# Edresson/VoiceSplit

Hardware: AMD Instinct MI355X
Metric: utterances/sec (3 s clips, B=64/GPU) fwd+bwd, channels-last bf16 activations / tape, bf16 MFMA, fp32 accumulate / statistics / master weights (higher is better)
Workload: dtype bf16 (conv activations and tape stored as bf16; bf16 MFMA operands in the convs, the LSTM / head contractions and the BPTT, f16 operands in the forward recurrence; fp32 accumulate, BatchNorm statistics, gate arithmetic / cell state, loss head, master weights)

## Files before the change

### voicesplit_amd/csrc/conv_nhwc.hip

```cpp
#include <utility>

#include "vs_internal.h"

namespace {

typedef unsigned u4v __attribute__((ext_vector_type(4)));
typedef unsigned u2v __attribute__((ext_vector_type(2)));
typedef float f2v __attribute__((ext_vector_type(2)));
constexpr float kLog2e = 1.44269504088896340736f;
typedef __attribute__((address_space(3))) unsigned char lds_byte;
typedef __attribute__((address_space(3))) const u4v lds_u4v;


constexpr int STRIP = 32;
constexpr int NB = STRIP / 16;
constexpr int R = 8;
#ifndef VS_NHWC_SGB
#define VS_NHWC_SGB 0
#endif

struct NhwcConvArgs {
  const unsigned short* in;
  const unsigned short* wpk;
  const float* scale;
  const float* shift;
  unsigned short* out;
  double* bn_stats;
  const unsigned short* z2;
  const float* bn2_scale; const float* bn2_shift; const float* bn2_mean; const float* bn2_invstd;
  int B, T, F, dil;
  int nstrip, nseg, seg_rows, n_items;
  unsigned* turn;
};

__device__ __forceinline__ int swz(int p) { return ((p >> 1) & 3) << 1; }

template <int KT, int KF>
struct Geo {
  static constexpr int P = KT / 2, PF = KF / 2, H = KT - 1;
  static constexpr int NTAP = KT * KF;
  static constexpr int RWPX = STRIP + 2 * PF;
  static constexpr int CPR = (RWPX * 8 + 63) / 64;
  static constexpr int ROWB = CPR * 1024;
  static constexpr int WIN = R + H;
  static constexpr int WBUF = WIN * ROWB;
  static constexpr int LDS_BYTES = 2 * WBUF;
  static constexpr int UNITS = (WIN + 3) / 4;
};

struct Item { int b, cls, strip, o0, o1, in_end, ngroups; };

template <int KT, int KF, int ACT, bool STATS, bool DY = false>
struct ConvWalk {
  using G = Geo<KT, KF>;
  static constexpr int P = G::P, PF = G::PF, H = G::H, NTAP = G::NTAP;
  static constexpr unsigned kOob = 0x7FFFFFF0u;

  const NhwcConvArgs& a;
  int lane, wave, n, g;
  vs_bf16x8 wf[NTAP][2];
  f2v csc[2], csh[2], a1[2], a2[2];
  int boff[KF][2];
  unsigned vcol[NB];
  int vdma;
  __amdgpu_buffer_rsrc_t rout, rz;
  f32x4 cacc[3][NB];
  unsigned crow[3];
  unsigned cvcol[NB];
  float ccok[NB];
  __amdgpu_buffer_rsrc_t crout, crz;
  u2v zq3[3][NB];
  unsigned lds0;
  const lds_byte* smem;

  __device__ __forceinline__ ConvWalk(const NhwcConvArgs& a_, const lds_byte* smem_) : a(a_), smem(smem_) {
    const int tid = threadIdx.x;
    lane = tid & 63;
    wave = __builtin_amdgcn_readfirstlane(tid >> 6);
    n = lane & 15;
    g = lane >> 4;
    lds0 = (unsigned)(uintptr_t)smem_;
    const u4v* wp = reinterpret_cast<const u4v*>(a.wpk) + (size_t)wave * NTAP * 2 * 64 + lane;
#pragma unroll
    for (int tap = 0; tap < NTAP; ++tap)
#pragma unroll
      for (int kc = 0; kc < 2; ++kc) wf[tap][kc] = __builtin_bit_cast(vs_bf16x8, wp[(tap * 2 + kc) * 64]);
#pragma unroll
    for (int r = 0; r < 4; ++r) {
      const int ch = wave * 16 + g * 4 + r;
      csc[r >> 1][r & 1] = DY ? a.bn2_scale[ch] * kLog2e : a.scale[ch];
      csh[r >> 1][r & 1] = DY ? a.bn2_shift[ch] * kLog2e : a.shift[ch];
      a1[r >> 1][r & 1] = 0.f;
      a2[r >> 1][r & 1] = 0.f;
    }
#pragma unroll
    for (int df = 0; df < KF; ++df) {
      const int p = n + df;
      boff[df][0] = p * 128 + ((g ^ swz(p)) << 4);
      boff[df][1] = boff[df][0] ^ 64;
    }
#pragma unroll
    for (int j = 0; j < 3; ++j) {
      crow[j] = kOob;
#pragma unroll
      for (int nb2 = 0; nb2 < NB; ++nb2) { cacc[j][nb2] = f32x4{0.f, 0.f, 0.f, 0.f}; zq3[j][nb2] = u2v{0u, 0u}; }
    }
#pragma unroll
    for (int nb2 = 0; nb2 < NB; ++nb2) { cvcol[nb2] = kOob; ccok[nb2] = 0.f; }
    crout = __builtin_amdgcn_make_buffer_rsrc(reinterpret_cast<unsigned char*>(a.out), 0, 0, 0x00020000);
    crz = crout;
    {
      const int px = lane >> 3;
      vdma = (px - PF) * 128 + (((lane & 7) ^ swz(px)) << 4);
    }
  }

  __device__ __forceinline__ bool decode(int it, Item& r) const {
    r.strip = it % a.nstrip;
    const int t1 = it / a.nstrip;
    const int seg = t1 % a.nseg;
    const int t2 = t1 / a.nseg;
    r.cls = t2 % a.dil;
    r.b = t2 / a.dil;
    const int nk = r.cls < a.T ? (a.T - r.cls + a.dil - 1) / a.dil : 0;
    r.o0 = seg * a.seg_rows;
    r.o1 = min(nk, r.o0 + a.seg_rows);
    if (r.o0 >= r.o1) return false;
    r.in_end = nk;
    r.ngroups = (r.o1 - r.o0 + R - 1) / R;
    return true;
  }

  struct Batch {
    long long row0;
    int in_end, w_first, buf, live;
    unsigned v0, v1;
  };
  Batch bt;
  __device__ __forceinline__ void begin(Batch& bt, const Item& x, int w_first, int buf) const {
    bt.row0 = (long long)x.b * a.T + x.cls;
    bt.in_end = x.in_end; bt.w_first = w_first; bt.buf = buf; bt.live = 1;
    bt.v0 = (unsigned)(vdma + ((x.strip * STRIP) << 7));
    bt.v1 = bt.v0 + 1024u;
  }
  template <int J>
  __device__ __forceinline__ void row_unit(const Batch& bt) const {
    const int rho = wave + 4 * J;
    if (!bt.live || rho >= G::WIN) return;
    const int w = bt.w_first + rho;
    const bool ok = (w >= 0) & (w < bt.in_end);
    const unsigned long long p = reinterpret_cast<unsigned long long>(a.in) + (unsigned long long)(((bt.row0 + (long long)w * a.dil) * a.F) << 7);
    const u4v d = {(unsigned)p, (unsigned)(p >> 32) & 0xffffu, ok ? (unsigned)a.F * 128u : 0u, 0x00020000u};
    const unsigned dst = lds0 + (unsigned)(bt.buf * G::WBUF + rho * G::ROWB);
    unsigned keep;
    static_assert(G::CPR == 4 || G::CPR == 5, "a window row is 4 or 5 chunks");
    if (G::CPR == 5)
      asm volatile("s_mov_b32 %0, m0\n\ts_mov_b32 m0, %3\n\ts_nop 0\n\tbuffer_load_dwordx4 %1, %2, 0 offen lds\n\t"
                   "s_add_u32 m0, %3, 0x400\n\ts_nop 0\n\tbuffer_load_dwordx4 %4, %2, 0 offen lds\n\t"
                   "buffer_load_dwordx4 %4, %2, 0 offen offset:1024 lds\n\tbuffer_load_dwordx4 %4, %2, 0 offen offset:2048 lds\n\t"
                   "buffer_load_dwordx4 %4, %2, 0 offen offset:3072 lds\n\ts_mov_b32 m0, %0"
                   : "=&s"(keep) : "v"(bt.v0), "s"(d), "s"(dst), "v"(bt.v1) : "memory", "scc");
    else
      asm volatile("s_mov_b32 %0, m0\n\ts_mov_b32 m0, %3\n\ts_nop 0\n\tbuffer_load_dwordx4 %1, %2, 0 offen lds\n\t"
                   "s_add_u32 m0, %3, 0x400\n\ts_nop 0\n\tbuffer_load_dwordx4 %4, %2, 0 offen lds\n\t"
                   "buffer_load_dwordx4 %4, %2, 0 offen offset:1024 lds\n\tbuffer_load_dwordx4 %4, %2, 0 offen offset:2048 lds\n\ts_mov_b32 m0, %0"
                   : "=&s"(keep) : "v"(bt.v0), "s"(d), "s"(dst), "v"(bt.v1) : "memory", "scc");
  }
  template <int... Js>
  __device__ __forceinline__ void all_units(const Batch& bt, std::integer_sequence<int, Js...>) const { (row_unit<Js>(bt), ...); }
  __device__ __forceinline__ void fetch_all(const Batch& bt) const { all_units(bt, std::make_integer_sequence<int, G::UNITS>()); }

  __device__ __forceinline__ void begin_item(const Item& x) {
    const size_t ub = (size_t)x.b * a.T * a.F * 128;
    const unsigned bytes = (unsigned)a.T * a.F * 128;
    rout = __builtin_amdgcn_make_buffer_rsrc(reinterpret_cast<unsigned char*>(a.out) + ub, 0, bytes, 0x00020000);
    if (DY) rz = __builtin_amdgcn_make_buffer_rsrc(const_cast<unsigned char*>(reinterpret_cast<const unsigned char*>(a.z2)) + ub, 0, bytes, 0x00020000);
#pragma unroll
    for (int nb2 = 0; nb2 < NB; ++nb2) {
      const int col = x.strip * STRIP + nb2 * 16 + n;
      vcol[nb2] = col < a.F ? (unsigned)(col * 128 + wave * 32 + g * 8) : kOob;
    }
  }
  __device__ __forceinline__ unsigned row_offset(const Item& x, int k) const {
    unsigned off;
    asm("s_mul_i32 %0, %1, %2" : "=s"(off) : "s"(x.cls + k * a.dil), "s"(a.F * 128));
    return k < x.o1 ? off : kOob;
  }

  template <int RV>
  struct GroupState {
    f32x4 acc[RV][NB];
    vs_bf16x8 bq[3];
    f2v y[NB][2];
    float cok[NB], mk[NB];
    f2v tz, ty, tu, tn, tr, tw, tp, tq;
    u2v pk[NB];
    unsigned vb[KF][2];
    int ro;
  };
  static constexpr int NSTAGE = DY ? (ACT == VS_ACT_MISH ? 19 : 7) : ACT == VS_ACT_MISH ? 12 : ACT == VS_ACT_RELU ? 2 : STATS ? 4 : 1;
  static constexpr int NMICRO = (DY ? 1 : 0) + NB * 2 * NSTAGE + 2 * NB;

  template <int RV>
  __device__ __forceinline__ vs_bf16x8 frag(const GroupState<RV>& st, int gi) const {
    const int nb = gi % NB, kc = (gi / NB) % 2, df = (gi / (2 * NB)) % KF, i = gi / (2 * NB * KF);
    return __builtin_bit_cast(vs_bf16x8, *(lds_u4v*)(uintptr_t)(st.vb[df][kc] + (unsigned)(i * G::ROWB + nb * 2048)));
  }

  static __device__ __forceinline__ float i_fma(float a, float b, float c) { return __builtin_fmaf(a, b, c); }
  static __device__ __forceinline__ float i_mul(float a, float b) { return a * b; }
  static __device__ __forceinline__ float i_add(float a, float b) { return a + b; }
  static __device__ __forceinline__ float i_add2(float a) { return a + 2.0f; }
  static __device__ __forceinline__ float i_exp2(float a) { return __builtin_amdgcn_exp2f(a); }
  static __device__ __forceinline__ float i_rcp(float a) { return __builtin_amdgcn_rcpf(a); }
  static __device__ __forceinline__ float i_max0(float a) { return fmaxf(a, 0.f); }
  static __device__ __forceinline__ float i_min_20log2e(float a) { return fminf(a, 20.0f * kLog2e); }
  static __device__ __forceinline__ float i_min_20(float a) { return fminf(a, 20.0f); }
  static __device__ __forceinline__ float i_mul_log2e(float a) { return a * kLog2e; }
  static __device__ __forceinline__ float i_mul_4ln2(float a) { return a * (4.0f * 0.69314718055994530942f); }
  static __device__ __forceinline__ float i_bf_lo(unsigned u) { return __uint_as_float(u << 16); }
  static __device__ __forceinline__ float i_bf_hi(unsigned u) { return __uint_as_float(u & 0xffff0000u); }

  static constexpr int epi_rows(int RV) { return RV >= 4 ? RV : 3; }
  template <int RV, int IDX, int nb2, int e>
  __device__ __forceinline__ float acc_of(GroupState<RV>& st) const {
    if constexpr (IDX < 3) return cacc[IDX][nb2][e];
    else return st.acc[IDX - 3][nb2][e];
  }
  template <int RV, int IDX>
  __device__ __forceinline__ unsigned rowoff_of(const Item& x, const GroupState<RV>& st) const {
    if constexpr (IDX < 3) return crow[IDX];
    else return row_offset(x, st.ro + IDX - 3);
  }
  template <int IDX, int nb2>
  __device__ __forceinline__ unsigned vcol_of() const {
    if constexpr (IDX < 3) return cvcol[nb2];
    else return vcol[nb2];
  }
  template <int RV, int IDX, bool FLUSH>
  __device__ __forceinline__ void prefetch_z(const Item& x, GroupState<RV>& st) {
    constexpr int t = IDX + 2, P_ = epi_rows(RV);
    if constexpr (t == 2) {
#pragma unroll
      for (int nb2 = 0; nb2 < NB; ++nb2) zq3[2][nb2] = __builtin_bit_cast(u2v, __builtin_amdgcn_raw_buffer_load_b64(crz, cvcol[nb2], crow[2], 0));
    } else if constexpr (!FLUSH) {
      constexpr int row = t < P_ ? t - 3 : (RV >= 4 ? RV - 3 : 0) + (t - P_);
      const unsigned so = row_offset(x, st.ro + row);
#pragma unroll
      for (int nb2 = 0; nb2 < NB; ++nb2) zq3[t % 3][nb2] = __builtin_bit_cast(u2v, __builtin_amdgcn_raw_buffer_load_b64(rz, vcol[nb2], so, 0));
    }
  }

  template <int RV, int IDX, int q, bool FLUSH>
  __device__ __forceinline__ void epi(const Item& x, GroupState<RV>& st) {
    constexpr bool mish = ACT == VS_ACT_MISH;
    constexpr int Q0 = DY ? 1 : 0;
    constexpr bool carried = IDX < 3;
    constexpr int r = IDX - 3;
    if constexpr (DY && q == 0) {
      prefetch_z<RV, IDX, FLUSH>(x, st);
#pragma unroll
      for (int nb2 = 0; nb2 < NB; ++nb2) {
        if constexpr (carried) st.mk[nb2] = crow[IDX] != kOob ? ccok[nb2] : 0.f;
        else st.mk[nb2] = (st.ro + r < x.o1) ? st.cok[nb2] : 0.f;
      }
    } else if constexpr (q < Q0 + NB * 2 * NSTAGE) {
      constexpr int v = (q - Q0) / NSTAGE, sg = (q - Q0) % NSTAGE, nb2 = v / 2, pr = v % 2;
      const float acc0 = acc_of<RV, IDX, nb2, 2 * pr>(st), acc1 = acc_of<RV, IDX, nb2, 2 * pr + 1>(st);
      if constexpr (DY) {
        if constexpr (sg == 0) {
          const unsigned u = zq3[IDX % 3][nb2][pr];
          st.tz.x = i_bf_lo(u); st.tz.y = i_bf_hi(u);
        } else if constexpr (sg == 1) {
          st.ty.x = i_fma(st.tz.x, csc[pr].x, csh[pr].x); st.ty.y = i_fma(st.tz.y, csc[pr].y, csh[pr].y);
        } else if constexpr (mish) {
          if constexpr (sg == 2) { st.ty.x = i_min_20log2e(st.ty.x); st.ty.y = i_min_20log2e(st.ty.y); }
          else if constexpr (sg == 3) st.tu.x = i_exp2(st.ty.x);
          else if constexpr (sg == 4) st.tu.y = i_exp2(st.ty.y);
          else if constexpr (sg == 5) { st.tw.x = i_add2(st.tu.x); st.tw.y = i_add2(st.tu.y); }
          else if constexpr (sg == 6) { st.tn.x = i_mul(st.tu.x, st.tw.x); st.tn.y = i_mul(st.tu.y, st.tw.y); }
          else if constexpr (sg == 7) { st.tw.x = i_add2(st.tn.x); st.tw.y = i_add2(st.tn.y); }
          else if constexpr (sg == 8) st.tr.x = i_rcp(st.tw.x);
          else if constexpr (sg == 9) st.tr.y = i_rcp(st.tw.y);
          else if constexpr (sg == 10) { st.tp.x = i_fma(st.tu.x, st.tu.x, st.tu.x); st.tp.y = i_fma(st.tu.y, st.tu.y, st.tu.y); }
          else if constexpr (sg == 11) { st.tp.x = i_mul(st.tp.x, st.ty.x); st.tp.y = i_mul(st.tp.y, st.ty.y); }
          else if constexpr (sg == 12) { st.tq.x = i_mul_4ln2(st.tr.x); st.tq.y = i_mul_4ln2(st.tr.y); }
          else if constexpr (sg == 13) { st.tn.x = i_fma(st.tp.x, st.tq.x, st.tn.x); st.tn.y = i_fma(st.tp.y, st.tq.y, st.tn.y); }
          else if constexpr (sg == 14) { st.tw.x = i_mul(st.tr.x, st.tn.x); st.tw.y = i_mul(st.tr.y, st.tn.y); }
          else if constexpr (sg == 15) { st.ty.x = i_mul(acc0, st.tw.x); st.ty.y = i_mul(acc1, st.tw.y); }
          else if constexpr (sg == 16) { st.tp.x = i_mul(st.ty.x, st.mk[nb2]); st.tp.y = i_mul(st.ty.y, st.mk[nb2]); }
          else if constexpr (sg == 17) { a1[pr].x = i_add(a1[pr].x, st.tp.x); a1[pr].y = i_add(a1[pr].y, st.tp.y); }
          else {
            a2[pr].x = i_fma(st.tp.x, st.tz.x, a2[pr].x); a2[pr].y = i_fma(st.tp.y, st.tz.y, a2[pr].y);
            st.y[nb2][pr] = st.ty;
          }
        } else {
          if constexpr (sg == 2) st.ty.x = st.ty.x > 0.f ? acc0 : 0.f;
          else if constexpr (sg == 3) st.ty.y = st.ty.y > 0.f ? acc1 : 0.f;
          else if constexpr (sg == 4) { st.tp.x = i_mul(st.ty.x, st.mk[nb2]); st.tp.y = i_mul(st.ty.y, st.mk[nb2]); }
          else if constexpr (sg == 5) { a1[pr].x = i_add(a1[pr].x, st.tp.x); a1[pr].y = i_add(a1[pr].y, st.tp.y); }
          else {
            a2[pr].x = i_fma(st.tp.x, st.tz.x, a2[pr].x); a2[pr].y = i_fma(st.tp.y, st.tz.y, a2[pr].y);
            st.y[nb2][pr] = st.ty;
          }
        }
      } else {
        if constexpr (sg == 0) {
          st.y[nb2][pr].x = i_fma(acc0, csc[pr].x, csh[pr].x); st.y[nb2][pr].y = i_fma(acc1, csc[pr].y, csh[pr].y);
        } else if constexpr (mish) {
          if constexpr (sg == 1) { st.ty.x = i_min_20(st.y[nb2][pr].x); st.ty.y = i_min_20(st.y[nb2][pr].y); }
          else if constexpr (sg == 2) { st.ty.x = i_mul_log2e(st.ty.x); st.ty.y = i_mul_log2e(st.ty.y); }
          else if constexpr (sg == 3) st.tu.x = i_exp2(st.ty.x);
          else if constexpr (sg == 4) st.tu.y = i_exp2(st.ty.y);
          else if constexpr (sg == 5) { st.tw.x = i_add2(st.tu.x); st.tw.y = i_add2(st.tu.y); }
          else if constexpr (sg == 6) { st.tn.x = i_mul(st.tu.x, st.tw.x); st.tn.y = i_mul(st.tu.y, st.tw.y); }
          else if constexpr (sg == 7) { st.tw.x = i_add2(st.tn.x); st.tw.y = i_add2(st.tn.y); }
          else if constexpr (sg == 8) st.tr.x = i_rcp(st.tw.x);
          else if constexpr (sg == 9) st.tr.y = i_rcp(st.tw.y);
          else if constexpr (sg == 10) { st.tn.x = i_mul(st.tn.x, st.tr.x); st.tn.y = i_mul(st.tn.y, st.tr.y); }
          else { st.y[nb2][pr].x = i_mul(st.y[nb2][pr].x, st.tn.x); st.y[nb2][pr].y = i_mul(st.y[nb2][pr].y, st.tn.y); }
        } else if constexpr (ACT == VS_ACT_RELU) {
          st.y[nb2][pr].x = i_max0(st.y[nb2][pr].x); st.y[nb2][pr].y = i_max0(st.y[nb2][pr].y);
        } else if constexpr (STATS) {
          if constexpr (sg == 1) {
            const float m = (int(rowoff_of<RV, IDX>(x, st) != kOob) & int(vcol_of<IDX, nb2>() != kOob)) ? 1.f : 0.f;
            st.tp.x = i_mul(st.y[nb2][pr].x, m); st.tp.y = i_mul(st.y[nb2][pr].y, m);
          } else if constexpr (sg == 2) { a1[pr].x = i_add(a1[pr].x, st.tp.x); a1[pr].y = i_add(a1[pr].y, st.tp.y); }
          else { a2[pr].x = i_fma(st.tp.x, st.y[nb2][pr].x, a2[pr].x); a2[pr].y = i_fma(st.tp.y, st.y[nb2][pr].y, a2[pr].y); }
        }
      }
    } else {
      constexpr int sq = q - Q0 - NB * 2 * NSTAGE, nb2 = sq / 2;
      if constexpr (sq % 2 == 0) {
        st.pk[nb2] = u2v{vs_pack_bf16(st.y[nb2][0].x, st.y[nb2][0].y), vs_pack_bf16(st.y[nb2][1].x, st.y[nb2][1].y)};
      } else {
        if constexpr (carried) __builtin_amdgcn_raw_buffer_store_b64(st.pk[nb2], crout, cvcol[nb2], crow[IDX], 0);
        else __builtin_amdgcn_raw_buffer_store_b64(st.pk[nb2], rout, vcol[nb2], row_offset(x, st.ro + r), 0);
      }
    }
  }

  static constexpr int nm_of(int RV, int i) { return (i < RV - 1 ? i : RV - 1) - (i - (KT - 1) > 0 ? i - (KT - 1) : 0) + 1; }
  static constexpr int slot_base(int RV, int i) { int s = 0; for (int k = 0; k < i; ++k) s += 2 * NB * KF * nm_of(RV, k); return s; }
  template <int RV>
  struct Plan {
    static constexpr int NSLOT = slot_base(RV, RV + H);
    static constexpr int P_ = epi_rows(RV);
    static constexpr int L = P_ * NMICRO;
    struct Tab { short lo[NSLOT + 1]; };
    static constexpr Tab make() {
      Tab t{};
      int c = 0, s = 0;
      for (int i = 0; i < RV + H; ++i) {
        int rows = i - H;
        if (rows < 0) rows = 0;
        if (rows > P_ - 3) rows = P_ - 3;
        const int avail = (3 + rows) * NMICRO;
        for (int k = 0; k < 2 * NB * KF * nm_of(RV, i); ++k) {
          t.lo[s] = (short)c;
          const int left = NSLOT - s;
          int want = (L - c + left - 1) / left;
          if (want < 1) want = 1;
          int n = avail - c;
          if (n > want) n = want;
          if (n < 0) n = 0;
          c += n;
          ++s;
        }
      }
      t.lo[NSLOT] = (short)c;
      return t;
    }
    static constexpr Tab tab = make();
  };
  template <int RV, bool FLUSH, int M0, int... Ds>
  __device__ __forceinline__ void epis(const Item& x, GroupState<RV>& st, std::integer_sequence<int, Ds...>) {
    (epi<RV, (M0 + Ds) / NMICRO, (M0 + Ds) % NMICRO, FLUSH>(x, st), ...);
  }

  template <int RV, int GI, int MM>
  __device__ __forceinline__ void gmfma(const Item& x, GroupState<RV>& st) {
    constexpr int nb = GI % NB, kc = (GI / NB) % 2, df = (GI / (2 * NB)) % KF, i = GI / (2 * NB * KF), ls = GI % (2 * NB * KF);
    constexpr int r_lo = i - (KT - 1) > 0 ? i - (KT - 1) : 0, r_hi = i < RV - 1 ? i : RV - 1;
    constexpr int nm = r_hi - r_lo + 1;
    constexpr int r = r_lo + MM;
    constexpr bool first = (i == r) && df == 0 && kc == 0;
    if constexpr (first)
      asm volatile("v_mfma_f32_16x16x32_bf16 %0, %1, %2, 0" : "=&v"(st.acc[r][nb]) : "a"(wf[(i - r) * KF + df][kc]), "v"(st.bq[GI % 3]));
    else
      asm volatile("v_mfma_f32_16x16x32_bf16 %0, %1, %2, %0" : "+v"(st.acc[r][nb]) : "a"(wf[(i - r) * KF + df][kc]), "v"(st.bq[GI % 3]));
    if constexpr (MM == 0 && GI % 4 == 0 && GI / 4 < G::UNITS) row_unit<GI / 4>(bt);
    constexpr int sl = slot_base(RV, i) + ls * nm + MM;
    constexpr int m0 = Plan<RV>::tab.lo[sl], m1 = Plan<RV>::tab.lo[sl + 1];
    epis<RV, false, m0>(x, st, std::make_integer_sequence<int, m1 - m0>());
    __builtin_amdgcn_sched_barrier(0);
  }

  template <int RV, int GI, int... MMs>
  __device__ __forceinline__ void gmfmas(const Item& x, GroupState<RV>& st, std::integer_sequence<int, MMs...>) {
    (gmfma<RV, GI, MMs>(x, st), ...);
  }

  template <int RV, int GI>
  __device__ __forceinline__ void gstep(const Item& x, GroupState<RV>& st) {
    constexpr int NG = (RV + H) * KF * 2 * NB;
    constexpr int i = GI / (2 * NB * KF);
    constexpr int r_lo = i - (KT - 1) > 0 ? i - (KT - 1) : 0, r_hi = i < RV - 1 ? i : RV - 1;
    if constexpr (GI + 2 < NG) st.bq[(GI + 2) % 3] = frag<RV>(st, GI + 2);
    __builtin_amdgcn_sched_barrier(0);
    gmfmas<RV, GI>(x, st, std::make_integer_sequence<int, r_hi - r_lo + 1>());
  }

  template <int RV, int... GIs>
  __device__ __forceinline__ void gsteps(const Item& x, GroupState<RV>& st, std::integer_sequence<int, GIs...>) {
    (gstep<RV, GIs>(x, st), ...);
  }

  template <int RV>
  __device__ __forceinline__ void group(const Item& x, int ro, int buf) {
    static_assert((RV + H) * KF * 2 * NB >= 4 * G::UNITS, "every DMA row unit needs a step");
    using PL = Plan<RV>;
    GroupState<RV> st;
    st.ro = ro;
#pragma unroll
    for (int df = 0; df < KF; ++df)
#pragma unroll
      for (int kc = 0; kc < 2; ++kc) st.vb[df][kc] = lds0 + (unsigned)(buf * G::WBUF + boff[df][kc]);
    if constexpr (DY) {
#pragma unroll
      for (int nb2 = 0; nb2 < NB; ++nb2) st.cok[nb2] = (x.strip * STRIP + nb2 * 16 + n < a.F) ? 1.f : 0.f;
    }
    st.bq[0] = frag<RV>(st, 0);
    st.bq[1] = frag<RV>(st, 1);
    gsteps<RV>(x, st, std::make_integer_sequence<int, (RV + H) * KF * 2 * NB>());
    epis<RV, false, PL::tab.lo[PL::NSLOT]>(x, st, std::make_integer_sequence<int, PL::L - PL::tab.lo[PL::NSLOT]>());
    asm volatile("s_nop 15" : "+v"(st.acc[RV - 1][0]), "+v"(st.acc[RV - 1][NB - 1]));
    constexpr int first = RV >= 4 ? RV - 3 : 0;
#pragma unroll
    for (int j = 0; j < 3; ++j) {
      if (first + j < RV) {
        crow[j] = row_offset(x, st.ro + first + j);
#pragma unroll
        for (int nb2 = 0; nb2 < NB; ++nb2) cacc[j][nb2] = st.acc[first + j < RV ? first + j : 0][nb2];
      } else {
        crow[j] = kOob;
      }
    }
#pragma unroll
    for (int nb2 = 0; nb2 < NB; ++nb2) {
      cvcol[nb2] = vcol[nb2];
      if constexpr (DY) ccok[nb2] = st.cok[nb2];
    }
    crout = rout;
    if constexpr (DY) {
      crz = rz;
      constexpr int sh = PL::P_ % 3;
      if constexpr (sh != 0) {
        u2v tmp[3][NB];
#pragma unroll
        for (int k = 0; k < 3; ++k)
#pragma unroll
          for (int nb2 = 0; nb2 < NB; ++nb2) tmp[k][nb2] = zq3[(k + sh) % 3][nb2];
#pragma unroll
        for (int k = 0; k < 3; ++k)
#pragma unroll
          for (int nb2 = 0; nb2 < NB; ++nb2) zq3[k][nb2] = tmp[k][nb2];
      }
    }
  }

  __device__ __forceinline__ void flush_carry() {
    Item x{};
    GroupState<2> st;
    st.ro = 0;
    epis<2, true, 0>(x, st, std::make_integer_sequence<int, 3 * NMICRO>());
  }

  __device__ __forceinline__ void flush_stats() {
    if (!(STATS || DY) || a.bn_stats == nullptr) return;
    float s1[4], s2[4];
#pragma unroll
    for (int r = 0; r < 4; ++r) { s1[r] = a1[r >> 1][r & 1]; s2[r] = a2[r >> 1][r & 1]; }
#pragma unroll
    for (int r = 0; r < 4; ++r) {
#pragma unroll
      for (int o = 8; o > 0; o >>= 1) {
        s1[r] += __shfl_xor(s1[r], o, 64);
        s2[r] += __shfl_xor(s2[r], o, 64);
      }
    }
    const unsigned slot = blockIdx.x % VS_BN_STAT_SLOTS, rank_in_slot = blockIdx.x / VS_BN_STAT_SLOTS;
    unsigned* my_turn = a.turn ? a.turn + VS_TURN_SLOT + slot : nullptr;
    vs_turn_begin(my_turn, rank_in_slot);
    if (n == 0) {
      double* dst = a.bn_stats + (size_t)(blockIdx.x % VS_BN_STAT_SLOTS) * 128 + (wave * 16 + g * 4) * 2;
#pragma unroll
      for (int r = 0; r < 4; ++r) {
        double t1 = (double)s1[r], t2 = (double)s2[r];
        if (DY) {
          const int ch = wave * 16 + g * 4 + r;
          t2 = (double)a.bn2_invstd[ch] * (t2 - (double)a.bn2_mean[ch] * t1);
        }
        atomicAdd(dst + 2 * r, t1);
        atomicAdd(dst + 2 * r + 1, t2);
      }
    }
    vs_turn_end(my_turn, rank_in_slot, (gridDim.x - slot + VS_BN_STAT_SLOTS - 1) / VS_BN_STAT_SLOTS);
  }
};

template <int KT, int KF, int ACT, bool STATS, bool DY>
__device__ __forceinline__ void nhwc_conv_body(const NhwcConvArgs& a, const unsigned char* smem) {
  using G = Geo<KT, KF>;
  ConvWalk<KT, KF, ACT, STATS, DY> wk(a, (const lds_byte*)smem);

  Item pf;
  int pf_it = (int)blockIdx.x, pf_g = 0;
  bool pf_live = false;
  auto pf_seek = [&]() {
    pf_live = false;
    while (pf_it < a.n_items) {
      if (wk.decode(pf_it, pf)) { pf_g = 0; pf_live = true; return; }
      pf_it += (int)gridDim.x;
    }
  };
  int pbuf = 0;
  auto pf_begin = [&]() {
    wk.begin(wk.bt, pf, pf.o0 + pf_g * R - G::P, pbuf);
    pbuf ^= 1;
    if (++pf_g >= pf.ngroups) { pf_it += (int)gridDim.x; pf_seek(); }
  };
  wk.bt.live = 0;
  pf_seek();
  if (pf_live) { pf_begin(); wk.fetch_all(wk.bt); }

  Item cur;
  int cbuf = 0;
  for (int it = (int)blockIdx.x; it < a.n_items; it += (int)gridDim.x) {
    if (!wk.decode(it, cur)) continue;
    wk.begin_item(cur);
    for (int gidx = 0; gidx < cur.ngroups; ++gidx) {
      asm volatile("s_waitcnt vmcnt(0)" ::: "memory");
      __builtin_amdgcn_s_barrier();
      wk.bt.live = 0;
      if (pf_live) pf_begin();
      const int ro = cur.o0 + gidx * R;
      const int left = cur.o1 - ro;
      if (left > 6) wk.template group<8>(cur, ro, cbuf);
      else if (left > 4) wk.template group<6>(cur, ro, cbuf);
      else if (left > 2) wk.template group<4>(cur, ro, cbuf);
      else wk.template group<2>(cur, ro, cbuf);
      cbuf ^= 1;
    }
  }
  wk.flush_carry();
  wk.flush_stats();
}

template <int KT, int KF, int ACT, bool STATS, bool DY = false>
__global__ __launch_bounds__(256, 1) VS_NO_PACKED_FP32
void nhwc_conv_kernel(NhwcConvArgs a) {
  __shared__ __attribute__((aligned(16))) unsigned char smem[Geo<KT, KF>::LDS_BYTES];
  nhwc_conv_body<KT, KF, ACT, STATS, DY>(a, smem);
}

__global__ void nhwc_pack_kernel(const float* __restrict__ w, unsigned short* __restrict__ out, int KT, int KF, int transpose_flip) {
  const int ntap = KT * KF;
  const int total = 4 * ntap * 2 * 64 * 8;
  for (int i = blockIdx.x * blockDim.x + threadIdx.x; i < total; i += gridDim.x * blockDim.x) {
    const int j = i & 7, lane = (i >> 3) & 63, kc = (i >> 9) & 1;
    const int tap = (i >> 10) % ntap, q = (i >> 10) / ntap;
    const int m = 16 * q + (lane & 15), k = 32 * kc + 8 * (lane >> 4) + j;
    const int dt = tap / KF, df = tap - dt * KF;
    const float v = transpose_flip ? w[((size_t)(k * 64 + m) * KT + (KT - 1 - dt)) * KF + (KF - 1 - df)]
                                   : w[((size_t)(m * 64 + k) * KT + dt) * KF + df];
    out[i] = (unsigned short)(vs_pack_bf16(v, 0.f) & 0xffffu);
  }
}

int num_cus() {
  static int cus[16] = {0};
  int dev = 0;
  if (hipGetDevice(&dev) != hipSuccess || dev < 0 || dev >= 16) return 256;
  if (!cus[dev]) {
    int v = 0;
    if (hipDeviceGetAttribute(&v, hipDeviceAttributeMultiprocessorCount, dev) != hipSuccess || v <= 0) v = 256;
    cus[dev] = v;
  }
  return cus[dev];
}

template <int KT, int KF>
int launch_conv(NhwcConvArgs a, int act, hipStream_t stream) {
  const int nk_max = (a.T + a.dil - 1) / a.dil;
  const long long base_items = (long long)a.B * a.dil * a.nstrip;
  int nseg = (int)((4096 + base_items - 1) / base_items);
  if (nseg > nk_max / 16) nseg = nk_max / 16;
  if (nseg < 1) nseg = 1;
  int seg_rows = (nk_max + nseg - 1) / nseg;
  seg_rows = (seg_rows + R - 1) / R * R;
  nseg = (nk_max + seg_rows - 1) / seg_rows;
  a.nseg = nseg;
  a.seg_rows = seg_rows;
  const long long n_items = base_items * nseg;
  VS_REQUIRE(n_items < (1LL << 30), "nhwc conv: too many work items");
  a.n_items = (int)n_items;
  const int cus = num_cus();
  const dim3 grid((unsigned)(n_items < cus ? n_items : cus)), block(256);
  const size_t lds = 0;
  const bool stats = a.bn_stats != nullptr;
#define VS_NHWC_LAUNCH3(A, S, D) hipLaunchKernelGGL((nhwc_conv_kernel<KT, KF, A, S, D>), grid, block, lds, stream, a)
#define VS_NHWC_LAUNCH(A, S) VS_NHWC_LAUNCH3(A, S, false)
  if (a.z2) {
    VS_REQUIRE(stats && a.bn2_scale && a.bn2_shift && a.bn2_mean && a.bn2_invstd, "nhwc conv: the dy epilogue needs statistics slots and BatchNorm constants");
    if (act == VS_ACT_MISH) VS_NHWC_LAUNCH3(VS_ACT_MISH, false, true);
    else if (act == VS_ACT_RELU) VS_NHWC_LAUNCH3(VS_ACT_RELU, false, true);
    else VS_REQUIRE(false, "nhwc conv: dy epilogue for activation %d", act);
  } else if (stats) {
    VS_REQUIRE(act == VS_ACT_NONE, "nhwc conv: fused statistics go with no activation");
    VS_NHWC_LAUNCH(VS_ACT_NONE, true);
  } else if (act == VS_ACT_NONE) VS_NHWC_LAUNCH(VS_ACT_NONE, false);
  else if (act == VS_ACT_MISH) VS_NHWC_LAUNCH(VS_ACT_MISH, false);
  else if (act == VS_ACT_RELU) VS_NHWC_LAUNCH(VS_ACT_RELU, false);
  else VS_REQUIRE(false, "nhwc conv: unsupported activation %d", act);
#undef VS_NHWC_LAUNCH
#undef VS_NHWC_LAUNCH3
  VS_LAUNCH_CHECK();
  return 0;
}

}

size_t vs_nhwc_packed_bytes(int KT, int KF) { return (size_t)64 * 64 * KT * KF * 2; }

int vs_nhwc_pack_impl(const float* w, void* packed, int KT, int KF, int transpose_flip, hipStream_t stream) {
  VS_REQUIRE(w && packed, "nhwc pack: NULL argument");
  VS_REQUIRE((KT == 5 && KF == 5) || (KT == 7 && KF == 1), "nhwc pack: kernel %dx%d is not one of the stack's (7x1, 5x5)", KT, KF);
  hipLaunchKernelGGL(nhwc_pack_kernel, dim3(64), dim3(256), 0, stream, w, reinterpret_cast<unsigned short*>(packed), KT, KF, transpose_flip);
  VS_LAUNCH_CHECK();
  return 0;
}

int vs_nhwc_conv_impl(const void* in, const void* packed, const float* scale, const float* shift, void* out,
                      int B, int T, int F, int KT, int KF, int dil, int act, double* bn_stats, hipStream_t stream) {
  VS_REQUIRE(in && packed && scale && shift && out, "nhwc conv: NULL argument");
  VS_REQUIRE(B > 0 && T > 0 && F > 0 && dil > 0, "nhwc conv: bad shape B=%d T=%d F=%d dil=%d", B, T, F, dil);
  VS_REQUIRE((long long)T * F * 128 < 0x7F000000LL, "nhwc conv: an utterance of %d x %d pixels does not fit the 31-bit offsets of the epilogue", T, F);
  VS_REQUIRE((reinterpret_cast<uintptr_t>(in) & 15) == 0 && (reinterpret_cast<uintptr_t>(out) & 15) == 0 &&
             (reinterpret_cast<uintptr_t>(packed) & 15) == 0, "nhwc conv: buffers must be 16-byte aligned");
  NhwcConvArgs a{reinterpret_cast<const unsigned short*>(in), reinterpret_cast<const unsigned short*>(packed), scale, shift,
                 reinterpret_cast<unsigned short*>(out), bn_stats, nullptr, nullptr, nullptr, nullptr, nullptr,
                 B, T, F, dil, (F + STRIP - 1) / STRIP, 1, 0, 0, g_vs_turn};
  if (KT == 5 && KF == 5) return launch_conv<5, 5>(a, act, stream);
  if (KT == 7 && KF == 1) return launch_conv<7, 1>(a, act, stream);
  VS_REQUIRE(false, "nhwc conv: kernel %dx%d is not one of the stack's (7x1, 5x5)", KT, KF);
  return -1;
}

int vs_nhwc_conv_dy_impl(const void* dz, const void* packed, void* dy, const void* z, int act,
                         const float* bn_scale, const float* bn_shift, const float* bn_mean, const float* bn_invstd, double* bn_stats,
                         int B, int T, int F, int KT, int KF, int dil, hipStream_t stream) {
  VS_REQUIRE(dz && packed && dy && z && bn_scale && bn_shift && bn_mean && bn_invstd && bn_stats, "nhwc conv dy: NULL argument");
  VS_REQUIRE(B > 0 && T > 0 && F > 0 && dil > 0, "nhwc conv dy: bad shape B=%d T=%d F=%d dil=%d", B, T, F, dil);
  VS_REQUIRE((long long)T * F * 128 < 0x7F000000LL, "nhwc conv dy: an utterance of %d x %d pixels does not fit the 31-bit offsets of the epilogue", T, F);
  VS_REQUIRE((reinterpret_cast<uintptr_t>(dz) & 15) == 0 && (reinterpret_cast<uintptr_t>(dy) & 15) == 0 &&
             (reinterpret_cast<uintptr_t>(packed) & 15) == 0 && (reinterpret_cast<uintptr_t>(z) & 7) == 0, "nhwc conv dy: buffer alignment");
  NhwcConvArgs a{reinterpret_cast<const unsigned short*>(dz), reinterpret_cast<const unsigned short*>(packed), bn_scale, bn_shift,
                 reinterpret_cast<unsigned short*>(dy), bn_stats, reinterpret_cast<const unsigned short*>(z), bn_scale, bn_shift, bn_mean, bn_invstd,
                 B, T, F, dil, (F + STRIP - 1) / STRIP, 1, 0, 0, g_vs_turn};
  if (KT == 5 && KF == 5) return launch_conv<5, 5>(a, act, stream);
  if (KT == 7 && KF == 1) return launch_conv<7, 1>(a, act, stream);
  VS_REQUIRE(false, "nhwc conv dy: kernel %dx%d is not one of the stack's (7x1, 5x5)", KT, KF);
  return -1;
}
```

Measured before the change: 1458.

## Skip MFMA work for out-of-range halo rows in dilated 5-tap NHWC convs

Adds a GUARD variant of the NHWC conv walk that checks, at runtime, whether each halo window row at the top and bottom of a group lies inside the input. Rows that fall outside are skipped instead of running their MFMAs against zero padding; the skip still zeroes the accumulators, issues the DMA and prefetches the next fragments. The epilogue slot plan is rebuilt so epilogue micro-steps are spread only over unguarded slots, capped at two per slot. The guarded kernel is used for KT=5 when dilation is at least 8, and always on the dy path, where skipped padding rows are more common. The cost is runtime branches, extra code size, and a changed interleaving of epilogue work with MFMAs.

```diff
diff --git a/voicesplit_amd/csrc/conv_nhwc.hip b/voicesplit_amd/csrc/conv_nhwc.hip
--- a/voicesplit_amd/csrc/conv_nhwc.hip
+++ b/voicesplit_amd/csrc/conv_nhwc.hip
@@ -50,10 +50,11 @@
 
 struct Item { int b, cls, strip, o0, o1, in_end, ngroups; };
 
-template <int KT, int KF, int ACT, bool STATS, bool DY = false>
+template <int KT, int KF, int ACT, bool STATS, bool DY = false, bool GUARD = false>
 struct ConvWalk {
   using G = Geo<KT, KF>;
   static constexpr int P = G::P, PF = G::PF, H = G::H, NTAP = G::NTAP;
+  static_assert(!GUARD || G::P <= 2, "a guarded top row I holds the first product of output row I: the smallest group has two rows");
   static constexpr unsigned kOob = 0x7FFFFFF0u;
 
   const NhwcConvArgs& a;
@@ -342,6 +343,8 @@
 
   static constexpr int nm_of(int RV, int i) { return (i < RV - 1 ? i : RV - 1) - (i - (KT - 1) > 0 ? i - (KT - 1) : 0) + 1; }
   static constexpr int slot_base(int RV, int i) { int s = 0; for (int k = 0; k < i; ++k) s += 2 * NB * KF * nm_of(RV, k); return s; }
+  static constexpr bool guarded(int RV, int i) { return GUARD && (i < P || i >= RV + H - P); }
+  static constexpr int free_slots(int RV) { int s = 0; for (int k = 0; k < RV + H; ++k) if (!guarded(RV, k)) s += 2 * NB * KF * nm_of(RV, k); return s; }
   template <int RV>
   struct Plan {
     static constexpr int NSLOT = slot_base(RV, RV + H);
@@ -350,7 +353,7 @@
     struct Tab { short lo[NSLOT + 1]; };
     static constexpr Tab make() {
       Tab t{};
-      int c = 0, s = 0;
+      int c = 0, s = 0, f = 0;
       for (int i = 0; i < RV + H; ++i) {
         int rows = i - H;
         if (rows < 0) rows = 0;
@@ -358,14 +361,17 @@
         const int avail = (3 + rows) * NMICRO;
         for (int k = 0; k < 2 * NB * KF * nm_of(RV, i); ++k) {
           t.lo[s] = (short)c;
-          const int left = NSLOT - s;
+          ++s;
+          if (guarded(RV, i)) continue;
+          const int left = free_slots(RV) - f;
           int want = (L - c + left - 1) / left;
           if (want < 1) want = 1;
+          if (GUARD && want > 2) want = 2;
           int n = avail - c;
           if (n > want) n = want;
           if (n < 0) n = 0;
           c += n;
-          ++s;
+          ++f;
         }
       }
       t.lo[NSLOT] = (short)c;
@@ -411,9 +417,45 @@
     gmfmas<RV, GI>(x, st, std::make_integer_sequence<int, r_hi - r_lo + 1>());
   }
 
-  template <int RV, int... GIs>
-  __device__ __forceinline__ void gsteps(const Item& x, GroupState<RV>& st, std::integer_sequence<int, GIs...>) {
-    (gstep<RV, GIs>(x, st), ...);
+  static constexpr int FPR = 2 * NB * KF;
+  template <int RV, int I, int... Ls>
+  __device__ __forceinline__ void row_steps(const Item& x, GroupState<RV>& st, std::integer_sequence<int, Ls...>) {
+    (gstep<RV, I * FPR + Ls>(x, st), ...);
+  }
+
+  template <int RV, int I>
+  __device__ __forceinline__ void skip_row(GroupState<RV>& st) {
+    constexpr int NG = (RV + H) * FPR;
+    if constexpr (I < P) {
+#pragma unroll
+      for (int nb2 = 0; nb2 < NB; ++nb2) st.acc[I][nb2] = f32x4{0.f, 0.f, 0.f, 0.f};
+    }
+    if constexpr (I == 0) {
+      static_assert(4 * (G::UNITS - 1) < FPR, "the DMA row units hang on window row 0");
+      fetch_all(bt);
+    }
+    if constexpr ((I + 1) * FPR < NG) {
+      st.bq[((I + 1) * FPR) % 3] = frag<RV>(st, (I + 1) * FPR);
+      st.bq[((I + 1) * FPR + 1) % 3] = frag<RV>(st, (I + 1) * FPR + 1);
+    }
+    if constexpr (I < P) asm volatile("s_nop 7" : "+v"(st.acc[I][0]), "+v"(st.acc[I][NB - 1]));
+    __builtin_amdgcn_sched_barrier(0);
+  }
+
+  template <int RV, int I>
+  __device__ __forceinline__ void grow(const Item& x, GroupState<RV>& st) {
+    if constexpr (guarded(RV, I)) {
+      const int w = st.ro - P + I;
+      if ((w >= 0) & (w < x.in_end)) row_steps<RV, I>(x, st, std::make_integer_sequence<int, FPR>());
+      else skip_row<RV, I>(st);
+    } else {
+      row_steps<RV, I>(x, st, std::make_integer_sequence<int, FPR>());
+    }
+  }
+
+  template <int RV, int... Is>
+  __device__ __forceinline__ void grows(const Item& x, GroupState<RV>& st, std::integer_sequence<int, Is...>) {
+    (grow<RV, Is>(x, st), ...);
   }
 
   template <int RV>
@@ -432,10 +474,16 @@
     }
     st.bq[0] = frag<RV>(st, 0);
     st.bq[1] = frag<RV>(st, 1);
-    gsteps<RV>(x, st, std::make_integer_sequence<int, (RV + H) * KF * 2 * NB>());
+    grows<RV>(x, st, std::make_integer_sequence<int, RV + H>());
     epis<RV, false, PL::tab.lo[PL::NSLOT]>(x, st, std::make_integer_sequence<int, PL::L - PL::tab.lo[PL::NSLOT]>());
-    asm volatile("s_nop 15" : "+v"(st.acc[RV - 1][0]), "+v"(st.acc[RV - 1][NB - 1]));
     constexpr int first = RV >= 4 ? RV - 3 : 0;
+    if constexpr (GUARD && RV >= 4)
+      asm volatile("s_nop 15" : "+v"(st.acc[RV - 1][0]), "+v"(st.acc[RV - 1][NB - 1]), "+v"(st.acc[RV - 2][0]), "+v"(st.acc[RV - 2][NB - 1]),
+                                "+v"(st.acc[first][0]), "+v"(st.acc[first][NB - 1]));
+    else if constexpr (GUARD)
+      asm volatile("s_nop 15" : "+v"(st.acc[RV - 1][0]), "+v"(st.acc[RV - 1][NB - 1]), "+v"(st.acc[first][0]), "+v"(st.acc[first][NB - 1]));
+    else
+      asm volatile("s_nop 15" : "+v"(st.acc[RV - 1][0]), "+v"(st.acc[RV - 1][NB - 1]));
 #pragma unroll
     for (int j = 0; j < 3; ++j) {
       if (first + j < RV) {
@@ -509,10 +557,10 @@
   }
 };
 
-template <int KT, int KF, int ACT, bool STATS, bool DY>
+template <int KT, int KF, int ACT, bool STATS, bool DY, bool GUARD>
 __device__ __forceinline__ void nhwc_conv_body(const NhwcConvArgs& a, const unsigned char* smem) {
   using G = Geo<KT, KF>;
-  ConvWalk<KT, KF, ACT, STATS, DY> wk(a, (const lds_byte*)smem);
+  ConvWalk<KT, KF, ACT, STATS, DY, GUARD> wk(a, (const lds_byte*)smem);
 
   Item pf;
   int pf_it = (int)blockIdx.x, pf_g = 0;
@@ -557,11 +605,11 @@
   wk.flush_stats();
 }
 
-template <int KT, int KF, int ACT, bool STATS, bool DY = false>
+template <int KT, int KF, int ACT, bool STATS, bool DY = false, bool GUARD = false>
 __global__ __launch_bounds__(256, 1) VS_NO_PACKED_FP32
 void nhwc_conv_kernel(NhwcConvArgs a) {
   __shared__ __attribute__((aligned(16))) unsigned char smem[Geo<KT, KF>::LDS_BYTES];
-  nhwc_conv_body<KT, KF, ACT, STATS, DY>(a, smem);
+  nhwc_conv_body<KT, KF, ACT, STATS, DY, GUARD>(a, smem);
 }
 
 __global__ void nhwc_pack_kernel(const float* __restrict__ w, unsigned short* __restrict__ out, int KT, int KF, int transpose_flip) {
@@ -588,6 +636,26 @@
     cus[dev] = v;
   }
   return cus[dev];
+}
+
+#ifndef VS_NHWC_GUARD_MIN_DIL
+#define VS_NHWC_GUARD_MIN_DIL 8
+#endif
+#ifndef VS_NHWC_GUARD_MIN_DIL_DY
+#define VS_NHWC_GUARD_MIN_DIL_DY 1
+#endif
+
+template <int KT, int KF, int ACT, bool STATS, bool DY>
+void launch_instance(dim3 grid, dim3 block, hipStream_t stream, const NhwcConvArgs& a) {
+  constexpr int min_dil = DY ? VS_NHWC_GUARD_MIN_DIL_DY : VS_NHWC_GUARD_MIN_DIL;
+  constexpr bool can_guard = KT == 5;
+  if constexpr (can_guard) {
+    if (min_dil <= 1 || a.dil >= min_dil) {
+      hipLaunchKernelGGL((nhwc_conv_kernel<KT, KF, ACT, STATS, DY, true>), grid, block, 0, stream, a);
+      return;
+    }
+  }
+  if constexpr (!can_guard || min_dil > 1) hipLaunchKernelGGL((nhwc_conv_kernel<KT, KF, ACT, STATS, DY, false>), grid, block, 0, stream, a);
 }
 
 template <int KT, int KF>
@@ -607,9 +675,8 @@
   a.n_items = (int)n_items;
   const int cus = num_cus();
   const dim3 grid((unsigned)(n_items < cus ? n_items : cus)), block(256);
-  const size_t lds = 0;
   const bool stats = a.bn_stats != nullptr;
-#define VS_NHWC_LAUNCH3(A, S, D) hipLaunchKernelGGL((nhwc_conv_kernel<KT, KF, A, S, D>), grid, block, lds, stream, a)
+#define VS_NHWC_LAUNCH3(A, S, D) launch_instance<KT, KF, A, S, D>(grid, block, stream, a)
 #define VS_NHWC_LAUNCH(A, S) VS_NHWC_LAUNCH3(A, S, false)
   if (a.z2) {
     VS_REQUIRE(stats && a.bn2_scale && a.bn2_shift && a.bn2_mean && a.bn2_invstd, "nhwc conv: the dy epilogue needs statistics slots and BatchNorm constants");
```

After: 1469, median of 6. No clear change (+0.8%).
